# mittagessen/conformer_ocr

Measured on AMD Instinct MI355X. Metric: text lines/sec (whole node) + CER vs reference, 96×1200 bf16 batch, higher is better.
Workload: dtype bf16; 1 GPU; cfg2: conformer D=256 L=12 heads=4 sub_ch=256, batch 32 x 96x1200 per GPU, forward + CTC greedy; batches_in_queue=1, parallelism=1 independent rank(s), weights by one RCCL broadcast, streams_per_gpu=4, hipgraph_replay=True, launched_by=in-process, gpu_max_hw_queues=4, gpu_max_hw_queues_preset_by_caller=True

## Files before the change

conformer_ocr_amd/csrc/attention.hip.h:

```cpp
#pragma once
#include "common.hip.h"

__device__ __forceinline__ int xcd_remap_i(int bid, int nwg) {
    const int q = nwg >> 3, r = nwg & 7, xcd = bid & 7;
    return (xcd < r ? xcd * (q + 1) : r * (q + 1) + (xcd - r) * q) + (bid >> 3);
}

__device__ __forceinline__ float max3_f(float a, float b, float c) {
    float r;
    asm("v_max3_f32 %0, %1, %2, %3" : "=v"(r) : "v"(a), "v"(b), "v"(c));
    return r;
}

#define COCR_MFMA_WAIT "s_nop 7\n\ts_nop 7\n\ts_nop 3"
__device__ __forceinline__ void mfma_results_fence(f32x4 (&a)[4]) { asm volatile(COCR_MFMA_WAIT : "+v"(a[0]), "+v"(a[1]), "+v"(a[2]), "+v"(a[3])); }
__device__ __forceinline__ void mfma_results_fence(f32x4 (&a)[4], f32x4 (&b)[4]) {
    asm volatile(COCR_MFMA_WAIT : "+v"(a[0]), "+v"(a[1]), "+v"(a[2]), "+v"(a[3]), "+v"(b[0]), "+v"(b[1]), "+v"(b[2]), "+v"(b[3]));
}
__device__ __forceinline__ void mfma_results_fence(f32x4 (&a)[4], f32x4 (&b)[4], f32x4 (&c)[4]) {
    asm volatile(COCR_MFMA_WAIT : "+v"(a[0]), "+v"(a[1]), "+v"(a[2]), "+v"(a[3]), "+v"(b[0]), "+v"(b[1]), "+v"(b[2]), "+v"(b[3]), "+v"(c[0]), "+v"(c[1]), "+v"(c[2]),
                 "+v"(c[3]));
}

#ifndef COCR_ATT_EXP
// ... 385 lines not shown
                if (i0 + row < Tn) *reinterpret_cast<bf16x8 *>(ctx + ((size_t)b * Tn + i0 + row) * (heads * DHP) + hh * DHP + 8 * ch) = v8;
            }
            return;
        }
    }
    if (dh == DHP) {
        if (i0 + il < Tn) {
            T *dst = ctx + ((size_t)b * Tn + i0 + il) * (heads * DHP) + hh * DHP + 4 * g;
#pragma unroll
            for (int d = 0; d < DT; ++d) {
                const f32x4 r4 = o[d] * inv;
                if constexpr (sizeof(T) == 2) { bf16x4 w = {(T)r4[0], (T)r4[1], (T)r4[2], (T)r4[3]}; *reinterpret_cast<bf16x4 *>(dst + 16 * d) = w; }
                else { *reinterpret_cast<f32x4 *>(dst + 16 * d) = r4; }
            }
        }
    } else if (i0 + il < Tn) {
        T *dst = ctx + ((size_t)b * Tn + i0 + il) * (heads * dh) + hh * dh;
#pragma unroll
        for (int d = 0; d < DT; ++d) {
            const int dd = 16 * d + 4 * g;
            if (dd + 3 < dh && (dh & 3) == 0) {
                float r4[4] = {o[d][0] * inv, o[d][1] * inv, o[d][2] * inv, o[d][3] * inv};
                if constexpr (sizeof(T) == 2) { bf16x4 w = {(T)r4[0], (T)r4[1], (T)r4[2], (T)r4[3]}; *reinterpret_cast<bf16x4 *>(dst + dd) = w; }
                else { *reinterpret_cast<f32x4 *>(dst + dd) = (f32x4){r4[0], r4[1], r4[2], r4[3]}; }
            } else {
#pragma unroll
                for (int r = 0; r < 4; ++r)
                    if (dd + r < dh) dst[dd + r] = from_f32<T>(o[d][r] * inv);
            }
        }
    }
}


constexpr int AF_QT = 10;
constexpr int AF_TK = 320;
constexpr int AF_SK = 20;
#ifndef COCR_AF_TWOPART
#define COCR_AF_TWOPART 1
#endif
constexpr int AF_WAVES = 8;
constexpr int AF_SROWS = 32;
constexpr size_t AF_LDS = (size_t)(2 * AF_TK + 16 * AF_QT + AF_TK) * 128 + AF_WAVES * AF_SROWS * AF_SK * sizeof(float);
static_assert(AF_LDS <= 160 * 1024, "LDS of the resident attention kernel");

struct AttnFullState {
    bf16x8 qu[2][2], qv[2][2];
    f32x4 o[2][4], osum[2];
    float m_run[2];
};

template <int NT>
__device__ __forceinline__ void attn_full_tiles(const unsigned char *ks, const unsigned char *vs, const unsigned char *ps, float *sk,
                                                AttnFullState &st, int lb_first, int Tn, int Tk, int kg0, int lane, bool sync_after_first = false) {
    typedef bf16_t T;
    constexpr int KC = 2, DT = 4, RS = 128;
    const int il = lane & 15, g = lane >> 4;
    const int fo0 = ((g ^ (il & 7)) << 4), fo1 = (((4 + g) ^ (il & 7)) << 4);
    auto &qu = st.qu;
    auto &qv = st.qv;
    auto &o = st.o;
    auto &osum = st.osum;
    auto &m_run = st.m_run;
    bf16x8 ones;
#pragma unroll
    for (int j = 0; j < 8; ++j) ones[j] = il == 0 ? (T)1.0f : (T)0.0f;

    for (int j0 = 0; j0 < Tk; j0 += 64) {
        const bool first_tile = kg0 + j0 == 0;
        f32x4 sc[NT][4], keep[NT];
#pragma unroll
        for (int half = 0; half < 2; ++half) {
            const int js = j0 + 32 * half;
            bf16x8 bfr[NT + 2][KC];
            {
                const unsigned char *pb0 = ps + (size_t)(lb_first - 16 * (NT - 1) + js + il) * RS;
#pragma unroll
                for (int u = 0; u < NT + 2; ++u) {
                    if (half == 1 && u == 0) continue;
                    bfr[u][0] = *reinterpret_cast<const bf16x8 *>(pb0 + u * 16 * RS + fo0);
                    bfr[u][1] = *reinterpret_cast<const bf16x8 *>(pb0 + u * 16 * RS + fo1);
                }
            }
#pragma unroll
            for (int t = 0; t < NT; ++t) {
                const f32x4 negm = {-m_run[t], -m_run[t], -m_run[t], -m_run[t]};
#pragma unroll
                for (int ml = 0; ml < 3; ++ml) {
                    f32x4 rr;
                    if (half == 1 && ml == 0) rr = keep[t];
                    else {
                        rr = negm;
#pragma unroll
                        for (int c = 0; c < KC; ++c) rr = mma16(bfr[ml + (NT - 1 - t)][c], qv[t][c], rr);
                    }
                    if (half == 0 && ml == 2) keep[t] = rr;
#pragma unroll
                    for (int r = 0; r < 4; ++r) sk[((16 * ml + 4 * g + r) & (AF_SROWS - 1)) * AF_SK + il] = rr[r];
                    if (ml >= 1) {
#pragma unroll
                        for (int r = 0; r < 4; ++r) sc[t][2 * half + ml - 1][r] = sk[((15 - il + 16 * (ml - 1) + 4 * g + r) & (AF_SROWS - 1)) * AF_SK + il];
                    }
                }
            }
            bf16x8 kf[2][KC];
#pragma unroll
            for (int tl = 0; tl < 2; ++tl) {
                const unsigned char *kr = ks + (size_t)(js + 16 * tl + il) * RS;
                kf[tl][0] = *reinterpret_cast<const bf16x8 *>(kr + fo0);
                kf[tl][1] = *reinterpret_cast<const bf16x8 *>(kr + fo1);
            }
#pragma unroll
            for (int t = 0; t < NT; ++t)
#pragma unroll
                for (int tl = 0; tl < 2; ++tl)
#pragma unroll
                    for (int c = 0; c < KC; ++c) sc[t][2 * half + tl] = mma16(kf[tl][c], qu[t][c], sc[t][2 * half + tl]);
        }
        bf16x8 pb[NT][2];
        if constexpr (NT == 1) mfma_results_fence(sc[0]);
        else if constexpr (NT == 2) mfma_results_fence(sc[0], sc[1]);
// ... 51 lines not shown
                    for (int r = 0; r < 4; ++r) sc[t][tt][r] -= delta;
            }
        }
#pragma unroll
        for (int t = 0; t < NT; ++t) {
#pragma unroll
            for (int tt = 0; tt < 4; ++tt)
#pragma unroll
                for (int r = 0; r < 4; ++r) pb[t][tt >> 1][4 * (tt & 1) + r] = (T)__builtin_amdgcn_exp2f(sc[t][tt][r]);
            osum[t] = mma16(ones, pb[t][0], osum[t]);
            osum[t] = mma16(ones, pb[t][1], osum[t]);
        }
#pragma unroll
        for (int d = 0; d < DT; ++d) {
            const bf16x8 v0 = load_vt_frag<true>(vs, RS, j0, d, il, g, T()), v1 = load_vt_frag<true>(vs, RS, j0 + 32, d, il, g, T());
#pragma unroll
            for (int t = 0; t < NT; ++t) {
                o[t][d] = mma16(v0, pb[t][0], o[t][d]);
                o[t][d] = mma16(v1, pb[t][1], o[t][d]);
            }
        }
        if (j0 == 0 && sync_after_first) {
            asm volatile("s_waitcnt vmcnt(0)" ::: "memory");
            __builtin_amdgcn_s_barrier();
        }
    }
}

template <int NT>
__device__ __forceinline__ void attn_full_store(float *sk, const AttnFullState &st, bf16_t *ctxh, int ctx_stride, int i_first, int Tn, int lane) {
    typedef bf16_t T;
    constexpr int DT = 4;
    const int il = lane & 15, g = lane >> 4;
    auto &o = st.o;
    auto &osum = st.osum;
    unsigned char *stg = reinterpret_cast<unsigned char *>(sk);
#pragma unroll
    for (int t = 0; t < NT; ++t) {
        const float inv = 1.0f / __shfl(osum[t][0], il, 64);
#pragma unroll
        for (int d = 0; d < DT; ++d) {
            const f32x4 r4 = o[t][d] * inv;
            const bf16x4 w = {(T)r4[0], (T)r4[1], (T)r4[2], (T)r4[3]};
            *reinterpret_cast<bf16x4 *>(stg + il * 128 + (((2 * d + (g >> 1)) ^ (il & 7)) << 4) + 8 * (g & 1)) = w;
        }
#pragma unroll
        for (int j = 0; j < 2; ++j) {
            const int row = 8 * j + (lane >> 3), ch = lane & 7;
            const bf16x8 v8 = *reinterpret_cast<const bf16x8 *>(stg + row * 128 + ((ch ^ (row & 7)) << 4));
            const int i = i_first + 16 * t + row;
            if (i < Tn) *reinterpret_cast<bf16x8 *>(ctxh + (size_t)i * ctx_stride + 8 * ch) = v8;
        }
    }
}

template <bool LONG>
__global__ __launch_bounds__(64 * AF_WAVES) void relpos_attention_full_kernel(const bf16_t *__restrict__ q, const bf16_t *__restrict__ k, const bf16_t *__restrict__ v,
                                                                    const bf16_t *__restrict__ ptab, const float *__restrict__ ub,
                                                                    const float *__restrict__ vb, bf16_t *__restrict__ ctx,
                                                                    int Tn, int Tp, int heads, float scale, int pos_center, int ntw, int kpass) {
    typedef bf16_t T;
    extern __shared__ __attribute__((aligned(16))) unsigned char att_smem[];
    const int Tk = (Tn + 63) & ~63;
    const int Kp = min(kpass, Tk);
    const int nbr = 16 * ntw + Kp;
    unsigned char *ks = att_smem, *vs = ks + (size_t)Kp * 128, *ps = vs + (size_t)Kp * 128;
    float *skew = reinterpret_cast<float *>(ps + (size_t)nbr * 128);
    const int tid = threadIdx.x, lane = tid & 63;
    const int wave = __builtin_amdgcn_readfirstlane(tid >> 6);
    const int nqb = gridDim.x, logical = xcd_remap_i(blockIdx.x + nqb * blockIdx.y, nqb * gridDim.y);
    const int qb = logical % nqb, bh = logical / nqb, b = bh / heads, hh = bh - b * heads;
    const int i0 = qb * 16 * ntw;
    const int nt_here = min(ntw, (Tn - i0 + 15) >> 4);
    static_assert(AF_QT <= 2 * AF_WAVES, "at most two query tiles per wave");
    const int base = nt_here / AF_WAVES, extra = nt_here % AF_WAVES;
    const int mine = base + (wave < extra ? 1 : 0), first = wave * base + min(wave, extra);
    const int i_first = i0 + 16 * first;
    bf16x8 qq[2][2];
    f32x4 u4[2][2], v4[2][2];
    {
        const int il = lane & 15, g = lane >> 4;
        const T *qrows = q + (size_t)bh * Tp * 64;
#pragma unroll
        for (int t = 0; t < 2; ++t) {
            const int iq = min(i_first + 16 * min(t, max(mine - 1, 0)) + il, Tn - 1);
#pragma unroll
            for (int c = 0; c < 2; ++c) qq[t][c] = load_frag(qrows + (size_t)iq * 64 + c * 32 + 8 * g);
        }
#pragma unroll
        for (int c = 0; c < 2; ++c)
#pragma unroll
            for (int hlf = 0; hlf < 2; ++hlf) {
                u4[c][hlf] = *reinterpret_cast<const f32x4 *>(ub + hh * 64 + c * 32 + 8 * g + 4 * hlf);
                v4[c][hlf] = *reinterpret_cast<const f32x4 *>(vb + hh * 64 + c * 32 + 8 * g + 4 * hlf);
            }
    }
    auto stage = [&](int kg0, int a, int b2) {
        const int r8 = lane >> 3, cs = lane & 7, gch = (cs ^ r8) * 8;
        const T *kb = k + ((size_t)bh * Tp + kg0) * 64, *vbs = v + ((size_t)bh * Tp + kg0) * 64;
        for (int rg = a / 8 + wave; rg < b2 / 8; rg += AF_WAVES) {
            __builtin_amdgcn_global_load_lds((gbl_ptr_t)(kb + (size_t)(rg * 8 + r8) * 64 + gch), (lds_ptr_t)(ks + rg * 1024), 16, 0, 0);
            __builtin_amdgcn_global_load_lds((gbl_ptr_t)(vbs + (size_t)(rg * 8 + r8) * 64 + gch), (lds_ptr_t)(vs + rg * 1024), 16, 0, 0);
        }
        const int prow = heads * 64;
        const T *pb = ptab + (size_t)(pos_center - i0 - (16 * ntw - 1) + kg0) * prow + hh * 64;
        for (int rg = (a ? (16 * ntw + a) / 8 : 0) + wave; rg < (16 * ntw + b2) / 8; rg += AF_WAVES)
            __builtin_amdgcn_global_load_lds((gbl_ptr_t)(pb + (size_t)(rg * 8 + r8) * prow + gch), (lds_ptr_t)(ps + rg * 1024), 16, 0, 0);
    };
    stage(0, 0, (!LONG && COCR_AF_TWOPART) ? min(64, Kp) : Kp);
    AttnFullState st;
#pragma unroll
    for (int t = 0; t < 2; ++t) {
#pragma unroll
        for (int c = 0; c < 2; ++c)
#pragma unroll
            for (int j = 0; j < 8; ++j) {
                const float x = (float)qq[t][c][j];
                st.qu[t][c][j] = (T)((x + u4[c][j >> 2][j & 3]) * scale);
                st.qv[t][c][j] = (T)((x + v4[c][j >> 2][j & 3]) * scale);
            }
        st.osum[t] = (f32x4){0.f, 0.f, 0.f, 0.f};
        st.m_run[t] = 0.f;
#pragma unroll
        for (int d = 0; d < 4; ++d) st.o[t][d] = (f32x4){0.f, 0.f, 0.f, 0.f};
    }
    const int lb_first = 16 * ntw - 16 - 16 * first;
    float *sk = skew + wave * AF_SROWS * AF_SK;
    if constexpr (!LONG) {
        const bool two = COCR_AF_TWOPART && Kp > 64;
        asm volatile("s_waitcnt vmcnt(0)" ::: "memory");
        __builtin_amdgcn_s_barrier();
        if (two) stage(0, 64, Kp);
        if (mine == 0) {
            if (two) { asm volatile("s_waitcnt vmcnt(0)" ::: "memory"); __builtin_amdgcn_s_barrier(); }
            return;
        }
        T *ctxh = ctx + (size_t)b * Tn * (heads * 64) + hh * 64;
        if (mine == 1) { attn_full_tiles<1>(ks, vs, ps, sk, st, lb_first, Tn, Kp, 0, lane, two); attn_full_store<1>(sk, st, ctxh, heads * 64, i_first, Tn, lane); }
        else { attn_full_tiles<2>(ks, vs, ps, sk, st, lb_first, Tn, Kp, 0, lane, two); attn_full_store<2>(sk, st, ctxh, heads * 64, i_first, Tn, lane); }
        return;
    }
    for (int kg0 = 0; kg0 < Tk; kg0 += Kp) {
        const int kn = min(Kp, Tk - kg0);
        if (kg0 > 0) {
            __builtin_amdgcn_s_barrier();
            stage(kg0, 0, kn);
        }
        asm volatile("s_waitcnt vmcnt(0)" ::: "memory");
        __builtin_amdgcn_s_barrier();
        if (mine == 1) attn_full_tiles<1>(ks, vs, ps, sk, st, lb_first, Tn, kn, kg0, lane);
        else if (mine == 2) attn_full_tiles<2>(ks, vs, ps, sk, st, lb_first, Tn, kn, kg0, lane);
    }
    T *ctxh = ctx + (size_t)b * Tn * (heads * 64) + hh * 64;
    if (mine == 1) attn_full_store<1>(sk, st, ctxh, heads * 64, i_first, Tn, lane);
    else if (mine == 2) attn_full_store<2>(sk, st, ctxh, heads * 64, i_first, Tn, lane);
}

template <typename T, int DHP> static inline size_t attention_lds_bytes() {
    const size_t rb = DHP * sizeof(T);
    return (size_t)(64 + 64 + 128) * ((rb == 128 && sizeof(T) == 2) ? rb : rb + 16) + 4 * 48 * 20 * sizeof(float);
}
```

conformer_ocr_amd/csrc/cocr_api.hip:

```cpp
#include <hip/hip_runtime.h>

#include <algorithm>
#include <cmath>
#include <cstdarg>
#include <cstdio>
#include <cstdlib>
#include <cstring>
#include <map>
#include <string>
#include <thread>
#include <vector>

#include "../../include/cocr.h"
#include "attention.hip.h"
#include "common.hip.h"
#include "conv.hip.h"
#include "ctc.hip.h"
#include "ctc_loss.hip.h"
#include "train.hip.h"
#include "train_enc.hip.h"
#include "gemm.hip.h"
#include "ffn.hip.h"
#include "rowchain_args.hip.h"
#include "pack.hip.h"
// ... 93 lines not shown
    int dtype = -1;
    unsigned char *blob = nullptr;
    BlobPlan plan;
    unsigned char *packed = nullptr;
    bf16_t *fpack = nullptr;
    bool packed_stale = true;
    unsigned char *ptab = nullptr;
    size_t ptab_stride = 0;
    bool ptab_stale = true;
    cocr_model *owner = nullptr;
    unsigned long long wgen = 1, seen_wgen = 0;
    int capN = 0, capW = 0;
    std::vector<void *> ws_allocs;
    void *z_a = nullptr, *z_b = nullptr;
    float *x = nullptr;
    void *g_lines = nullptr;
    float *g_logits = nullptr;
    void *xn = nullptr, *hid = nullptr, *q = nullptr, *k = nullptr, *vt = nullptr, *ctx = nullptr, *glu = nullptr, *dwo = nullptr;
    size_t qkv_bytes = 0;
    int vtN = -1, vtT = -1;
    int pos_maxlen = COCR_POS_MAXLEN;
    DevBuf<unsigned char> pre_buf;
    DevBuf<unsigned char> page_buf;
    DevBuf<int32_t> d_lens, h_lens{true};
    int32_t *d_lens_cur = nullptr;
    int lens_slot = 0;
    DevBuf<int32_t> ctc_lab;
    DevBuf<float> ctc_val;
    const float *amax_logits = nullptr;
    int amax_rows = 0;
    bool amax_ok = false;
    DevBuf<float> tr_pad;
    DevBuf<unsigned char> beam_bp;
    DevBuf<int32_t> loss_d, loss_h{true};
    int loss_slot = 0;
    DevBuf<float> loss_ws;
    DevBuf<unsigned char> score_d, score_h{true};
    hipEvent_t score_ev[4] = {nullptr, nullptr, nullptr, nullptr};
    int score_slot = 0;
    DevBuf<unsigned> score_ws;
    int score_lds_max = 64 * 1024;
    int lastN = 0, lastT = 0;
    DevBuf<float> tr_part;
    float *tr_state = nullptr;
    long tr_step = 0;
    bool use_graph = false;
    struct GraphEntry { const void *lines; float *logits; int N, W, dtype; hipStream_t s; hipGraphExec_t exec; };
    std::vector<GraphEntry> graphs, graph_seen;
    bool debug = false;
    unsigned long long *stamps = nullptr;
    bool no_pad = false;
    bool beam_ref = false;
    bool no_front96 = false;
    bool no_front32 = false;
    bool no_dw_fuse = false;
    int chain_rows = 0;
    bool no_front_chain = false;
    bool ffn_probe = false;
    int att_resident_min = 192;
    bool att_resident_long = false;
    bool att_tiled = false;
    bool no_kskip = false;
    bool chain_xcd = true;
    bool no_chain = false;
    std::map<std::string, std::pair<float *, int64_t>> taps;
    DevBuf<float> tapbuf;
    TrainState *train = nullptr;
    bool profile = false;
    std::vector<ProfRec> prof;
    std::vector<hipEvent_t> ev_pool;
};

static const char *FAMILIES[] = {"frontend_fused", "frontend_conv12", "frontend_dw", "gemm_front_pw", "gemm_front_out", "layernorm",
                                 "gemm_ffn_up", "gemm_ffn_down", "ffn_fused", "chain_ffn_qkv", "chain_front_ffn_qkv", "chain_attn_out_glu", "chain_pw2_ffn_ffn_qkv", "chain_pw2_ffn", "gemm_qkv", "attention", "gemm_attn_out", "gemm_glu",
                                 "dwconv", "gemm_pw2", "gemm_decoder", "ctc_greedy", "ctc_beam", "ctc_loss", "ffn_probe", "event_pair_overhead"};
enum { FAM_FRONT96, FAM_CONV12, FAM_FDW, FAM_FPW, FAM_FOUT, FAM_LN, FAM_FFN_UP, FAM_FFN_DOWN, FAM_FFN_FUSED, FAM_CH_FIRST, FAM_CH_FRONT, FAM_CH_A, FAM_CH_B, FAM_CH_LAST, FAM_QKV, FAM_ATTN, FAM_AOUT, FAM_GLU,
       FAM_DW, FAM_PW2, FAM_DEC, FAM_GREEDY, FAM_BEAM, FAM_LOSS, FAM_FFN_PROBE, FAM_EMPTY, FAM_COUNT };

static void drop_graphs(cocr_model *m) {
    for (auto &g : m->graphs) (void)hipGraphExecDestroy(g.exec);
    m->graphs.clear();
    m->graph_seen.clear();
}

static int out_len1(int l) { return l >= 1 ? (l - 1) / 2 + 1 : 0; }

extern "C" int32_t cocr_out_len(int32_t in_len, int32_t subsampling_factor) {
    int n = 0;
    for (int f = subsampling_factor; f > 1; f >>= 1) ++n;
    for (int i = 0; i < n; ++i) in_len = out_len1(in_len);
    return in_len;
}

static void add_name(cocr_model *m, const std::string &n) { m->names.push_back(n); m->host[n]; }

struct Switch { const char *name; bool cocr_model::*flag; int cocr_model::*count; };
static const Switch SWITCHES[] = {
    {"COCR_NO_PAD", &cocr_model::no_pad, nullptr},
    {"COCR_NO_CHAIN", &cocr_model::no_chain, nullptr},
    {"COCR_NO_FRONT_CHAIN", &cocr_model::no_front_chain, nullptr},
    {"COCR_FFN_PROBE", &cocr_model::ffn_probe, nullptr},
    {"COCR_ATT_TILED", &cocr_model::att_tiled, nullptr},
    {"COCR_ATT_RESIDENT_LONG", &cocr_model::att_resident_long, nullptr},
    {"COCR_CHAIN_XCD", &cocr_model::chain_xcd, nullptr},
    {"COCR_NO_KSKIP", &cocr_model::no_kskip, nullptr},
    {"COCR_NO_DW_FUSE", &cocr_model::no_dw_fuse, nullptr},
    {"COCR_NO_FRONT96", &cocr_model::no_front96, nullptr},
    {"COCR_NO_FRONT32", &cocr_model::no_front32, nullptr},
    {"COCR_BEAM_REF", &cocr_model::beam_ref, nullptr},
    {"COCR_ATT_RESIDENT_MIN", nullptr, &cocr_model::att_resident_min},
    {"COCR_CHAIN_ROWS", nullptr, &cocr_model::chain_rows},
    {"COCR_SCORE_LDS_MAX", nullptr, &cocr_model::score_lds_max},
};

extern "C" int cocr_create(const cocr_hparams *hp, int device, cocr_model **out) {
    if (!hp || !out) return fail(COCR_EINVAL, "null argument");
    if (hp->num_classes < 1 || hp->height < 1 || hp->encoder_dim < 1 || hp->num_encoder_layers < 1 || hp->num_attention_heads < 1)
        return fail(COCR_EINVAL, "non-positive hyper-parameter");
    if (hp->encoder_dim % hp->num_attention_heads) return fail(COCR_EINVAL, "d_model %% num_heads should be zero.");
    if ((hp->conv_kernel_size - 1) % 2 || hp->conv_kernel_size < 1) return fail(COCR_EINVAL, "kernel_size should be a odd number for 'SAME' padding");
    if (hp->conv_expansion_factor != 2) return fail(COCR_EINVAL, "Currently, Only Supports expansion_factor 2");
    int sf = hp->subsampling_factor, snum = 0;
    if (sf < 2 || (sf & (sf - 1))) return fail(COCR_EINVAL, "Sampling factor should be a power of 2.");
    for (int f = sf; f > 1; f >>= 1) ++snum;
    if (snum < 1) return fail(COCR_EINVAL, "subsampling_factor must be at least 2");
    if (hp->encoder_dim % 16) return fail(COCR_EUNSUPPORTED, "encoder_dim must be a multiple of 16 (GLU tile pairing, 16-byte rows)");
    if (hp->subsampling_conv_channels % 8) return fail(COCR_EUNSUPPORTED, "subsampling_conv_channels must be a multiple of 8");
    if (hp->encoder_dim > COCR_LN_MAX_D) return fail(COCR_EUNSUPPORTED, "encoder_dim > 1024");
    const int dh = hp->encoder_dim / hp->num_attention_heads;
    if (dh > 128) return fail(COCR_EUNSUPPORTED, "d_head > 128");
    cocr_model *m = new cocr_model();
    m->hp = *hp;
    m->device = device;
    m->D = hp->encoder_dim; m->C = hp->subsampling_conv_channels; m->L = hp->num_encoder_layers;
    m->heads = hp->num_attention_heads; m->dh = dh; m->dhp = round_up(dh, 32);
    m->ff = hp->feed_forward_expansion_factor * hp->encoder_dim; m->ksz = hp->conv_kernel_size;
    m->rD = m->D; m->rff = m->ff; m->rdh = m->dh;
    m->ncls = hp->num_classes; m->H = hp->height; m->snum = snum;
    for (const Switch &w : SWITCHES) {
        const char *e = getenv(w.name);
        if (!e) continue;
        if (w.count) m->*w.count = atoi(e);
        else m->*w.flag = m->*w.flag ? e[0] != '0' : e[0] == '1';
    }
    { const char *e = getenv("COCR_CHAIN_STAMPS"); if (e && e[0] == '1') { (void)hipHostMalloc((void **)&m->stamps, 4096 * 8); memset(m->stamps, 0, 4096 * 8); } }
    int f = hp->height;
    for (int i = 0; i < snum; ++i) { f = out_len1(f); m->feats.push_back(f); }
    char buf[256];
    add_name(m, "encoder.conv_subsample.conv.0.weight");
    add_name(m, "encoder.conv_subsample.conv.0.bias");
    for (int s = 0, idx = 2; s < snum - 1; ++s, idx += 3) {
        for (int j = 0; j < 2; ++j) {
            snprintf(buf, sizeof buf, "encoder.conv_subsample.conv.%d.weight", idx + j); add_name(m, buf);
            snprintf(buf, sizeof buf, "encoder.conv_subsample.conv.%d.bias", idx + j); add_name(m, buf);
        }
    }
    add_name(m, "encoder.conv_subsample.out.0.weight");
    add_name(m, "encoder.conv_subsample.out.0.bias");
    for (int l = 0; l < m->L; ++l) {
        auto nm = [&](const char *suffix) { snprintf(buf, sizeof buf, "encoder.layers.%d.sequential.%s", l, suffix); add_name(m, buf); };
// ... 660 lines not shown
template <typename T> struct Fwd {
    cocr_model *m;
    const Form &f;
    hipStream_t s;
    const BlobPlan &P;
    const int N, W, D, T1, T2, F1, F2, Tn, M, Tp;
    const float ffr, scale;
    T *const za, *const zb;
    float *const x;
    T *const xn, *const hid, *const q, *const k, *const v, *const ctx, *const glu, *const dwo;
    Fwd(cocr_model *m_, const Form &f_, int N_, int W_, hipStream_t s_)
        : m(m_), f(f_), s(s_), P(m_->plan), N(N_), W(W_), D(m_->D), T1(out_len1(W_)), T2(m_->snum == 1 ? T1 : out_len1(T1)), F1(m_->feats[0]),
          F2(m_->feats[m_->snum == 1 ? 0 : 1]), Tn(cocr_out_len(W_, m_->hp.subsampling_factor)), M(N_ * Tn), Tp(round_up(Tn, 64)),
          ffr(m_->hp.half_step_residual ? 0.5f : 1.0f), scale(1.0f / sqrtf((float)m_->rdh)), za((T *)m_->z_a), zb((T *)m_->z_b), x(m_->x),
          xn((T *)m_->xn), hid((T *)m_->hid), q((T *)m_->q), k((T *)m_->k), v((T *)m_->vt), ctx((T *)m_->ctx), glu((T *)m_->glu), dwo((T *)m_->dwo) {}
    const float *F32(size_t off) const { return (const float *)(m->blob + off); }
    const T *WT(size_t off) const { return (const T *)(m->blob + off); }
    template <typename S> int tap(int l, const char *what, const S *src, size_t n) const {
        if (!f.taps) return COCR_OK;
        char nm[64];
        if (l < 0) snprintf(nm, sizeof nm, "%s", what);
        else snprintf(nm, sizeof nm, "l%d.%s", l, what);
        return ::tap<S>(m, s, nm, src, n);
    }
    int tap_x(int l, const char *what, const float *src) const { return tap<float>(l, what, src, (size_t)M * D); }
    int tap_qkv(int l) const {
        const size_t n = m->qkv_bytes / sizeof(T);
        int rc;
        if ((rc = tap<T>(l, "q", q, n)) || (rc = tap<T>(l, "k", k, n)) || (rc = tap<T>(l, "v", v, n))) return rc;
        return COCR_OK;
    }
};

template <typename T, typename TIn> static int frontend(const Fwd<T> &c, const TIn *lines) {
    cocr_model *m = c.m;
    const BlobPlan &P = c.P;
    const hipStream_t s = c.s;
    const int N = c.N, H = m->H, W = c.W, C = m->C, T1 = c.T1, F1 = c.F1, T2 = c.T2, F2 = c.F2;
    const FrontForm form = c.f.front;
    T *za = c.za, *zb = c.zb;
    int rc;
    if (form == FRONT_CONV0) {
        ProfScope ps(m, s, FAM_CONV12);
        const size_t npos = (size_t)N * T1 * F1;
        hipLaunchKernelGGL((frontend_conv0_kernel<T, TIn>), dim3((unsigned)((npos * (size_t)(C / 2) + 255) / 256)), dim3(256), 0, s, lines, H, W, T1, F1, C, npos,
                           c.F32(P.w0), c.F32(P.b0), zb);
        LAUNCH_CHECK();
        return COCR_OK;
    }
    if (form == FRONT_96) {
        ProfScope ps(m, s, FAM_FRONT96);
        const size_t n0 = (size_t)(C / 16) * 64 * 4;
        GEMM_TRY(launch_frontend96<TIn>(s, lines, N, H, W, T1, F1, T2, m->fpack, c.F32(P.b0), m->fpack + n0, c.F32(P.stages[0].dw_b),
                                        (const bf16_t *)(m->packed + P.stages[0].pw_w), c.F32(P.stages[0].pw_b), (bf16_t *)zb, m->stamps ? m->stamps + 128 : nullptr));
    } else if (form == FRONT_PW32) {
        ProfScope ps(m, s, FAM_CONV12);
        const size_t lds = (size_t)(4 * 16 + 3) * ((H + 11) & ~3) * 4 + (size_t)16 * F2 * 80;
        auto kern = frontend_conv12pw32_kernel<TIn>;
        GEMM_TRY(raise_lds_limit((const void *)kern, lds));
        hipLaunchKernelGGL(kern, dim3(ceil_div(T2, 16), N), dim3(256), lds, s, lines, H, W, T1, F1, T2, F2, c.F32(P.w0), c.F32(P.b0),
                           c.F32(P.stages[0].dw_w), c.F32(P.stages[0].dw_b), (const bf16_t *)c.WT(P.stages[0].pw_w), c.F32(P.stages[0].pw_b), (bf16_t *)zb);
        LAUNCH_CHECK();
    } else {
        {
            ProfScope ps(m, s, FAM_CONV12);
            if (form == FRONT_MFMA) {
                GEMM_TRY(launch_conv12_mfma<TIn>(s, lines, N, H, W, T1, F1, T2, F2, C, c.F32(P.w0), c.F32(P.b0), c.F32(P.stages[0].dw_w), c.F32(P.stages[0].dw_b),
                                                 (bf16_t *)za));
            } else {
                const int TB = std::max(1, 512 / C);
                const size_t lds = (size_t)(4 * TB + 3) * ((H + 11) & ~3) * 4;
                hipLaunchKernelGGL((frontend_conv12_kernel<T, TIn>), dim3(ceil_div(T2, TB), N), dim3(256), lds, s, lines, H, W, T1, F1, T2, F2, C,
                                   c.F32(P.w0), c.F32(P.b0), c.F32(P.stages[0].dw_w), c.F32(P.stages[0].dw_b), za, TB);
                LAUNCH_CHECK();
            }
        }
        if ((rc = c.tap(-1, "front.z2", za, (size_t)N * T2 * F2 * C))) return rc;
        ProfScope ps(m, s, FAM_FPW);
        EpiBiasAct<T, ACT_RELU> epi{zb, C, c.F32(P.stages[0].pw_b), C};
        GEMM_TRY(launch_gemm<T>(s, za, C, c.WT(P.stages[0].pw_w), C, N * T2 * F2, C, C, epi));
    }
    if ((rc = c.tap(-1, "front.z3", zb, (size_t)N * T2 * F2 * C))) return rc;
    int Tc = T2, Fc = F2;
    for (int st = 1; st < m->snum - 1; ++st) {
        const int To = out_len1(Tc), Fo = m->feats[st + 1];
        {
            ProfScope ps(m, s, FAM_FDW);
            hipLaunchKernelGGL((dw3x3s2_kernel<T>), dim3(1024), dim3(256), 0, s, zb, N, Tc, Fc, To, Fo, C, c.F32(P.stages[st].dw_w),
                               c.F32(P.stages[st].dw_b), za);
            LAUNCH_CHECK();
        }
        {
            ProfScope ps(m, s, FAM_FPW);
            EpiBiasAct<T, ACT_RELU> epi{zb, C, c.F32(P.stages[st].pw_b), C};
            GEMM_TRY(launch_gemm<T>(s, za, C, c.WT(P.stages[st].pw_w), C, N * To * Fo, C, C, epi));
        }
        Tc = To; Fc = Fo;
    }
    return COCR_OK;
}

template <typename T> static int layernorm(const Fwd<T> &c, size_t g1, size_t b1, bool write_f32, long g2, long b2) {
    ProfScope ps(c.m, c.s, FAM_LN);
    launch_layernorm<T>(c.s, c.x, c.M, c.D, c.F32(g1), c.F32(b1), write_f32 ? c.x : nullptr, g2 >= 0 ? c.F32((size_t)g2) : nullptr,
                        b2 >= 0 ? c.F32((size_t)b2) : nullptr, c.xn, c.m->rD);
    LAUNCH_CHECK();
    return COCR_OK;
// ... 993 lines not shown
```

conformer_ocr_amd/csrc/frontend.hip.h:

```cpp
#pragma once
#include "gemm.hip.h"
#include "conv.hip.h"

__global__ __launch_bounds__(256) void frontend_pack_kernel(const float *__restrict__ w0, const float *__restrict__ w2, bf16_t *__restrict__ w0f,
                                                            bf16_t *__restrict__ dwf, int C) {
    const int i = blockIdx.x * 256 + threadIdx.x;
    if (i < (C / 16) * 64 * 4) {
        const int e = i & 3, lane = (i >> 2) & 63, nt = i >> 8, r = lane & 15, g = lane >> 4;
        w0f[i] = (bf16_t)((g < 3 && e < 3) ? w0[(16 * nt + r) * 9 + 3 * g + e] : 0.0f);
    }
    if (i < (C / 16) * 5 * 64 * 8) {
        const int e = i & 7, lane = (i >> 3) & 63, chunk = (i >> 9) % 5, blk = i / (5 * 512), r = lane & 15, g = lane >> 4;
        const int tap = 2 * chunk + (g >> 1), cc = 8 * (g & 1) + e;
        dwf[i] = (bf16_t)((cc == r && tap < 9) ? w2[(16 * blk + r) * 9 + tap] : 0.0f);
    }
}

typedef unsigned u32x2_t __attribute__((ext_vector_type(2)));
__device__ __forceinline__ unsigned relu_pack2(float a, float b) {
    typedef short s16x2_t __attribute__((ext_vector_type(2)));
    typedef float f32x2_t __attribute__((ext_vector_type(2)));
    const bf16x2 h = __builtin_convertvector((f32x2_t){a, b}, bf16x2);
    const s16x2_t zero = {0, 0};
    return __builtin_bit_cast(unsigned, __builtin_elementwise_max(__builtin_bit_cast(s16x2_t, h), zero));
}
__device__ __forceinline__ u32x2_t relu_bf16x4(const f32x4 &v) { return (u32x2_t){relu_pack2(v[0], v[1]), relu_pack2(v[2], v[3])}; }

template <typename TIn>
__global__ __launch_bounds__(512) void frontend96_kernel(const TIn *__restrict__ X, int H, int W, int T1, int F1, int Tn,
                                                         const bf16_t *__restrict__ w0f, const float *__restrict__ b0,
                                                         const bf16_t *__restrict__ dwf, const float *__restrict__ b2,
                                                         const bf16_t *__restrict__ wpw,
                                                         const float *__restrict__ bpw, bf16_t *__restrict__ Z3, int HS, int N, unsigned long long *stamps) {
    typedef bf16_t T;
    constexpr int C = 256, F = 24, TB = 4, BMC = TB * F, MT = 6, KC1 = C / 32;
    constexpr int NA = 2 * TB + 1, NCOL = 4 * TB + 4, ZR = 2 * F + 2, ZC = 72;
    constexpr int PANEL = BMC * 128, IMG = 4 * PANEL, OS = C * 2 + 16, SLICE = 16 * 512;
    constexpr int XAB = BMC * OS > IMG ? BMC * OS : IMG;
    static_assert(BMC == 96, "operand image of the chain kernels");
    extern __shared__ __attribute__((aligned(16))) unsigned char smem[];
    unsigned char *xa = smem;
    T *z1 = reinterpret_cast<T *>(smem + XAB);
    T *xs = z1 + (NA * ZR + 1) * ZC;
    unsigned char *prm = reinterpret_cast<unsigned char *>(xs + NCOL * HS);
    const T *w0s = reinterpret_cast<const T *>(prm);
    const float *b0s = reinterpret_cast<const float *>(prm + 8192), *b2s = b0s + 256;

    const int tid = threadIdx.x, lane = tid & 63;
    const int wave = __builtin_amdgcn_readfirstlane(tid >> 6);
    const int r16 = lane & 15, g = lane >> 4, swz = r16 & 7;
    const int nblk = (Tn + TB - 1) / TB, nitems = nblk * N, stride = gridDim.x;
    int item = blockIdx.x;
#ifdef COCR_CHAIN_STAMPS_BUILD
    int nstamp = 0;
    auto stamp = [&]() {
        if (stamps && blockIdx.x == 1 && tid == 0 && nstamp < 40) stamps[nstamp] = __builtin_readcyclecounter();
        ++nstamp;
    };
#else
    auto stamp = [&]() {};
#endif
    stamp();

    constexpr int FILL = 4;
    TIn fv[FILL];
    auto load_pixels = [&](int it) {
        const int bb = it / nblk, c0 = 4 * (it - bb * nblk) * TB - 3;
        const TIn *Xb = X + (size_t)bb * H * W;
        int tv = tid;
        asm volatile("" : "+v"(tv));
#pragma unroll
        for (int u = 0; u < FILL; ++u) {
            const int i = tv + 512 * u, rr = i / NCOL, ci = i - rr * NCOL;
            const int w = min(max(c0 + ci, 0), W - 1), r = min(max(rr - 1, 0), H - 1);
            fv[u] = Xb[(size_t)r * W + w];
        }
    };
    if (item < nitems) load_pixels(item);
    __builtin_amdgcn_global_load_lds((gbl_ptr_t)(w0f + wave * 512 + lane * 8), (lds_ptr_t)(prm + wave * 1024), 16, 0, 0);
    if (wave < 2) __builtin_amdgcn_global_load_lds((gbl_ptr_t)((wave ? b2 : b0) + lane * 4), (lds_ptr_t)(prm + 8192 + wave * 1024), 16, 0, 0);
    asm volatile("s_waitcnt vmcnt(0)" ::: "memory");
    const int FT = (F1 + 15) >> 4, ntile = NA * FT;
    const int blk = wave & 3, mq = wave >> 2;

    for (; item < nitems; item += stride) {
    const int b = item / nblk, t0 = (item - b * nblk) * TB;
    int tv = tid;
    asm volatile("" : "+v"(tv));
    bf16x8 ring[16];
    for (int i = tv; i < NA * ZC; i += 512) {
        const int a = i / ZC, c = i - a * ZC;
        z1[(a * ZR) * ZC + c] = (T)0.0f;
        for (int zr = F1 + 1; zr < ZR; ++zr) z1[(a * ZR + zr) * ZC + c] = (T)0.0f;
    }
#pragma unroll
    for (int u = 0; u < FILL; ++u) {
        const int i = tv + 512 * u, rr = i / NCOL, ci = i - rr * NCOL, c = 4 * t0 - 3 + ci;
        const bool inside = c >= 0 && c < W && rr >= 1 && rr <= H;
        if (i < NCOL * HS) xs[ci * HS + rr] = (T)(inside ? pixel_to_f32<TIn>(fv[u]) : 0.0f);
    }
    stamp();
    asm volatile("s_waitcnt lgkmcnt(0)" ::: "memory");
    __builtin_amdgcn_s_barrier();
    stamp();

    s16x4 pf[4];
    bool valid[4];
    int zoff[4];
#pragma unroll
    for (int u = 0; u < 4; ++u) {
        const int mt = min(wave + 8 * u, ntile - 1);
        const int a = mt / FT, f1 = 16 * (mt - a * FT) + r16;
        const int t1 = 2 * t0 - 1 + a;
        const T *px = xs + (2 * a + g) * HS + 2 * f1;
        typedef unsigned u32x2 __attribute__((ext_vector_type(2)));
        pf[u] = __builtin_bit_cast(s16x4, (u32x2){*reinterpret_cast<const unsigned *>(px), *reinterpret_cast<const unsigned *>(px + 2)});
        valid[u] = t1 >= 0 && t1 < T1 && f1 < F1;
        zoff[u] = (wave + 8 * u < ntile && f1 + 1 < ZR) ? (a * ZR + f1 + 1) * ZC : NA * ZR * ZC;
    }
    const bool all_valid = __builtin_amdgcn_ballot_w64(valid[0] && valid[1] && valid[2] && valid[3]) == ~0ull;
    bf16x8 dwn[5];
    auto request_dw = [&](int pass) {
#pragma unroll
        for (int ch = 0; ch < 5; ++ch) dwn[ch] = *reinterpret_cast<const bf16x8 *>(dwf + ((size_t)(4 * pass + blk) * 5 + ch) * 512 + lane * 8);
    };
    request_dw(0);
    auto do_pass = [&](int pass, auto LAST) {
        const int cb = 64 * pass;
        bf16x8 dwb[5];
#pragma unroll
        for (int ch = 0; ch < 5; ++ch) dwb[ch] = dwn[ch];
        if (pass < 3) request_dw(pass + 1);
        const f32x4 bias2 = *reinterpret_cast<const f32x4 *>(b2s + cb + 16 * blk + 4 * g);
        s16x4 wf[4];
        f32x4 bias0[4];
#pragma unroll
        for (int nt = 0; nt < 4; ++nt) {
            wf[nt] = *reinterpret_cast<const s16x4 *>(w0s + ((size_t)((cb >> 4) + nt) * 64 + lane) * 4);
            bias0[nt] = *reinterpret_cast<const f32x4 *>(b0s + cb + 16 * nt + 4 * g);
        }
        f32x4 c0[4][4];
#pragma unroll
        for (int u = 0; u < 4; ++u)
#pragma unroll
            for (int nt = 0; nt < 4; ++nt) c0[u][nt] = __builtin_amdgcn_mfma_f32_16x16x16bf16_1k(wf[nt], pf[u], bias0[nt], 0, 0, 0);
        auto z1_epilogue = [&](auto MASKED) {
#pragma unroll
            for (int u = 0; u < 4; ++u)
#pragma unroll
                for (int nt = 0; nt < 4; ++nt) {
                    typedef unsigned u32x2 __attribute__((ext_vector_type(2)));
                    u32x2 ob = relu_bf16x4(c0[u][nt]);
                    if (decltype(MASKED)::value && !valid[u]) ob = (u32x2){0u, 0u};
                    *reinterpret_cast<u32x2 *>(z1 + zoff[u] + 16 * nt + 4 * g) = ob;
                }
        };
        if (all_valid) z1_epilogue(std::false_type{}); else z1_epilogue(std::true_type{});
        if constexpr (decltype(LAST)::value) {
            const T *first = wpw + (size_t)wave * SLICE;
#pragma unroll
            for (int f = 0; f < 16; ++f) ring[f] = *reinterpret_cast<const bf16x8 *>(first + f * 512 + lane * 8);
            if (item + stride < nitems) load_pixels(item + stride);
        }
        stamp();
        asm volatile("s_waitcnt lgkmcnt(0)" ::: "memory");
        __builtin_amdgcn_s_barrier();
        stamp();
#pragma unroll
        for (int u = 0; u < 3; ++u) {
            const int p = 16 * (mq + 2 * u) + r16, tl = p / F, f = p - tl * F;
            f32x4 acc = bias2;
#pragma unroll
            for (int ch = 0; ch < 5; ++ch) {
                const int tap = min(2 * ch + (g >> 1), 8), dt = tap / 3, df = tap - 3 * dt;
                const bf16x8 za = *reinterpret_cast<const bf16x8 *>(z1 + ((2 * tl + dt) * ZR + 2 * f + df) * ZC + 16 * blk + 8 * (g & 1));
                acc = mma16(dwb[ch], za, acc);
            }
            const bf16x4 o = {(T)acc[0], (T)acc[1], (T)acc[2], (T)acc[3]};
            const int col = cb + 16 * blk + 4 * g;
            *reinterpret_cast<bf16x4 *>(xa + (col >> 6) * PANEL + p * 128 + ((((col & 63) >> 3) ^ (p & 7)) << 4) + ((col & 7) >> 2) * 8) = o;
        }
        stamp();
        asm volatile("s_waitcnt lgkmcnt(0)" ::: "memory");
        __builtin_amdgcn_s_barrier();
    };
#pragma unroll 1
    for (int pass = 0; pass < 3; ++pass) do_pass(pass, std::false_type{});
    do_pass(3, std::true_type{});

    const f32x4 bp0 = *reinterpret_cast<const f32x4 *>(bpw + 32 * wave + 4 * g), bp1 = *reinterpret_cast<const f32x4 *>(bpw + 32 * wave + 16 + 4 * g);
    f32x4 acc[MT][2];
#pragma unroll
    for (int i = 0; i < MT; ++i) { acc[i][0] = bp0; acc[i][1] = bp1; }
#pragma unroll
    for (int kk = 0; kk < KC1; ++kk) {
        bf16x8 a[MT];
#pragma unroll
        for (int i = 0; i < MT; ++i) a[i] = lds_frag_swz(xa + (kk >> 1) * PANEL + (16 * i + r16) * 128, kk & 1, g, swz, T());
#pragma unroll
        for (int j = 0; j < 2; ++j)
#pragma unroll
            for (int i = 0; i < MT; ++i) acc[i][j] = mma16(ring[2 * kk + j], a[i], acc[i][j]);
    }
    stamp();
    __builtin_amdgcn_s_barrier();
    unsigned char *tile = xa;
#pragma unroll
    for (int j = 0; j < 2; ++j)
#pragma unroll
        for (int i = 0; i < MT; ++i) {
            const int row = 16 * i + r16;
            typedef unsigned u32x2 __attribute__((ext_vector_type(2)));
            *reinterpret_cast<u32x2 *>(tile + row * OS + (32 * wave + 16 * j + 4 * g) * 2) = relu_bf16x4(acc[i][j]);
        }
    asm volatile("s_waitcnt lgkmcnt(0)" ::: "memory");
    __builtin_amdgcn_s_barrier();
    stamp();
    T *out = Z3 + ((size_t)b * Tn + t0) * F * C;
    for (int id = tv; id < BMC * 32; id += 512) {
        const int row = id >> 5, ch = id & 31;
        if (t0 + row / F < Tn) copy16(out + (size_t)row * C + ch * 8, reinterpret_cast<const T *>(tile + row * OS + ch * 16));
    }
    stamp();
    }
}

static inline bool frontend96_supported(int C, int F1, int F2, int H) { return C == 256 && F2 == 24 && F1 <= 2 * F2 && H <= 4 * F2; }

template <typename TIn>
static inline hipError_t launch_frontend96(hipStream_t s, const TIn *X, int N, int H, int W, int T1, int F1, int Tn, const bf16_t *w0f, const float *b0,
                                           const bf16_t *dwf, const float *b2, const bf16_t *wpw, const float *bpw, bf16_t *Z3, unsigned long long *stamps = nullptr) {
    const int FT = (F1 + 15) / 16, HS = 2 * 16 * FT + 4;
    const size_t z1b = (size_t)(9 * 50 + 1) * 72 * 2, tileb = (size_t)96 * (256 * 2 + 16);
    const size_t lds = std::max((size_t)4 * 96 * 128, tileb) + z1b + (size_t)20 * HS * 2 + 10240;
    auto kern = frontend96_kernel<TIn>;
    hipError_t e = raise_lds_limit((const void *)kern, lds + 4096);
    if (e != hipSuccess) return e;
    static int ncu = 0;
    if (!ncu) {
        int dev = 0;
        hipDeviceProp_t prop;
        if (hipGetDevice(&dev) != hipSuccess || hipGetDeviceProperties(&prop, dev) != hipSuccess) return hipErrorUnknown;
        ncu = prop.multiProcessorCount > 0 ? prop.multiProcessorCount : 256;
    }
    const int nitems = ((Tn + 3) / 4) * N;
    hipLaunchKernelGGL(kern, dim3(std::min(nitems, ncu)), dim3(512), lds, s, X, H, W, T1, F1, Tn, w0f, b0, dwf, b2, wpw, bpw, Z3, HS, N, stamps);
    return hipGetLastError();
}
```

Baseline: 34780 lines/s.

## Split unbalanced attention query tiles across waves and preload frontend pointwise weights

In the resident attention kernel, when a block has one or two extra query tiles beyond one per wave, idle waves process the first half of the key range for an extra tile. They hand their partial softmax state (o, osum, running max) through LDS with a workgroup-scope flag, and the owning wave finishes the remaining keys. This balances work across waves at the cost of spin-waiting and extra LDS traffic. Separately, the frontend kernel now loads the pointwise weight ring once before the item loop (optionally per item under a new env flag) and issues the next depthwise weight request after the z1 epilogue rather than before it.

```diff
diff --git a/conformer_ocr_amd/csrc/attention.hip.h b/conformer_ocr_amd/csrc/attention.hip.h
--- a/conformer_ocr_amd/csrc/attention.hip.h
+++ b/conformer_ocr_amd/csrc/attention.hip.h
@@ -461,7 +461,8 @@
 
 template <int NT>
 __device__ __forceinline__ void attn_full_tiles(const unsigned char *ks, const unsigned char *vs, const unsigned char *ps, float *sk,
-                                                AttnFullState &st, int lb_first, int Tn, int Tk, int kg0, int lane, bool sync_after_first = false) {
+                                                AttnFullState &st, int lb_first, int Tn, int Tk, int kg0, int lane, bool sync_after_first = false,
+                                                int jb = 0) {
     typedef bf16_t T;
     constexpr int KC = 2, DT = 4, RS = 128;
     const int il = lane & 15, g = lane >> 4;
@@ -475,7 +476,7 @@
 #pragma unroll
     for (int j = 0; j < 8; ++j) ones[j] = il == 0 ? (T)1.0f : (T)0.0f;
 
-    for (int j0 = 0; j0 < Tk; j0 += 64) {
+    for (int j0 = jb; j0 < Tk; j0 += 64) {
         const bool first_tile = kg0 + j0 == 0;
         f32x4 sc[NT][4], keep[NT];
 #pragma unroll
@@ -633,6 +634,26 @@
             if (i < Tn) *reinterpret_cast<bf16x8 *>(ctxh + (size_t)i * ctx_stride + 8 * ch) = v8;
         }
     }
+}
+
+constexpr int AF_HAND_FLAG = (AF_SROWS - 1) * AF_SK + 16;
+static_assert(AF_HAND_FLAG * sizeof(float) >= 2048 && AF_HAND_FLAG < AF_SROWS * AF_SK, "flag behind the store's staging rows, inside the tile");
+__host__ __device__ constexpr int af_give_tiles(int nkt) { return (nkt + 1) / 2; }
+__device__ __forceinline__ void attn_full_give(unsigned char *buf, float *flag, const AttnFullState &st, int lane) {
+#pragma unroll
+    for (int d = 0; d < 4; ++d) *reinterpret_cast<f32x4 *>(buf + d * 1024 + lane * 16) = st.o[0][d];
+    *reinterpret_cast<f32x4 *>(buf + 4096 + lane * 16) = st.osum[0];
+    *reinterpret_cast<float *>(buf + 5120 + lane * 4) = st.m_run[0];
+    __hip_atomic_store(reinterpret_cast<unsigned *>(flag), 1u, __ATOMIC_RELEASE, __HIP_MEMORY_SCOPE_WORKGROUP);
+}
+__device__ __forceinline__ void attn_full_take(const unsigned char *buf, float *flag, AttnFullState &st, int lane) {
+    while (__hip_atomic_load(reinterpret_cast<unsigned *>(flag), __ATOMIC_ACQUIRE, __HIP_MEMORY_SCOPE_WORKGROUP) != 1u) __builtin_amdgcn_s_sleep(4);
+#pragma unroll
+    for (int d = 0; d < 4; ++d) st.o[0][d] = *reinterpret_cast<const f32x4 *>(buf + d * 1024 + lane * 16);
+    st.osum[0] = *reinterpret_cast<const f32x4 *>(buf + 4096 + lane * 16);
+    st.m_run[0] = *reinterpret_cast<const float *>(buf + 5120 + lane * 4);
+#pragma unroll
+    for (int c = 0; c < 2; ++c) { st.qu[0][c] = st.qu[1][c]; st.qv[0][c] = st.qv[1][c]; }
 }
 
 template <bool LONG>
@@ -657,6 +678,9 @@
     const int base = nt_here / AF_WAVES, extra = nt_here % AF_WAVES;
     const int mine = base + (wave < extra ? 1 : 0), first = wave * base + min(wave, extra);
     const int i_first = i0 + 16 * first;
+    const bool hand = !LONG && COCR_AF_TWOPART && Kp > 64 && base == 1 && extra >= 1 && extra <= 2;
+    const bool giver = hand && wave >= 4 && wave < 4 + extra, taker = hand && wave >= 6 && wave < 6 + extra;
+    const int handed = taker ? (wave - 2) + extra : first;
     bf16x8 qq[2][2];
     f32x4 u4[2][2], v4[2][2];
     {
@@ -664,7 +688,7 @@
         const T *qrows = q + (size_t)bh * Tp * 64;
 #pragma unroll
         for (int t = 0; t < 2; ++t) {
-            const int iq = min(i_first + 16 * min(t, max(mine - 1, 0)) + il, Tn - 1);
+            const int iq = min((t == 1 && taker ? i0 + 16 * handed : i_first + 16 * min(t, max(mine - 1, 0))) + il, Tn - 1);
 #pragma unroll
             for (int c = 0; c < 2; ++c) qq[t][c] = load_frag(qrows + (size_t)iq * 64 + c * 32 + 8 * g);
         }
@@ -709,7 +733,9 @@
     float *sk = skew + wave * AF_SROWS * AF_SK;
     if constexpr (!LONG) {
         const bool two = COCR_AF_TWOPART && Kp > 64;
-        asm volatile("s_waitcnt vmcnt(0)" ::: "memory");
+        float *flag = skew + (taker ? wave - 2 : wave) * AF_SROWS * AF_SK + AF_HAND_FLAG;
+        if (giver && lane == 0) __hip_atomic_store(reinterpret_cast<unsigned *>(flag), 0u, __ATOMIC_RELAXED, __HIP_MEMORY_SCOPE_WORKGROUP);
+        asm volatile("s_waitcnt vmcnt(0) lgkmcnt(0)" ::: "memory");
         __builtin_amdgcn_s_barrier();
         if (two) stage(0, 64, Kp);
         if (mine == 0) {
@@ -717,9 +743,17 @@
             return;
         }
         T *ctxh = ctx + (size_t)b * Tn * (heads * 64) + hh * 64;
-        if (mine == 1) { attn_full_tiles<1>(ks, vs, ps, sk, st, lb_first, Tn, Kp, 0, lane, two); attn_full_store<1>(sk, st, ctxh, heads * 64, i_first, Tn, lane); }
-        else { attn_full_tiles<2>(ks, vs, ps, sk, st, lb_first, Tn, Kp, 0, lane, two); attn_full_store<2>(sk, st, ctxh, heads * 64, i_first, Tn, lane); }
-        return;
+        if (mine == 2) { attn_full_tiles<2>(ks, vs, ps, sk, st, lb_first, Tn, Kp, 0, lane, two); attn_full_store<2>(sk, st, ctxh, heads * 64, i_first, Tn, lane); return; }
+        const int jsplit = 64 * af_give_tiles(Kp >> 6);
+        unsigned char *hbuf = (giver ? wave - 4 : wave - 6) ? vs : ks;
+        for (int round = 0;; ++round) {
+            const int tile = round ? handed : first;
+            attn_full_tiles<1>(ks, vs, ps, sk, st, 16 * ntw - 16 - 16 * tile, Tn, giver ? jsplit : Kp, 0, lane, two && round == 0, round ? jsplit : 0);
+            if (giver) { attn_full_give(hbuf, flag, st, lane); return; }
+            attn_full_store<1>(sk, st, ctxh, heads * 64, i0 + 16 * tile, Tn, lane);
+            if (!taker || round) return;
+            attn_full_take(hbuf, flag, st, lane);
+        }
     }
     for (int kg0 = 0; kg0 < Tk; kg0 += Kp) {
         const int kn = min(Kp, Tk - kg0);
diff --git a/conformer_ocr_amd/csrc/cocr_api.hip b/conformer_ocr_amd/csrc/cocr_api.hip
--- a/conformer_ocr_amd/csrc/cocr_api.hip
+++ b/conformer_ocr_amd/csrc/cocr_api.hip
@@ -169,6 +169,7 @@
     bool no_pad = false;
     bool beam_ref = false;
     bool no_front96 = false;
+    bool front_ring = false;
     bool no_front32 = false;
     bool no_dw_fuse = false;
     int chain_rows = 0;
@@ -223,6 +224,7 @@
     {"COCR_NO_KSKIP", &cocr_model::no_kskip, nullptr},
     {"COCR_NO_DW_FUSE", &cocr_model::no_dw_fuse, nullptr},
     {"COCR_NO_FRONT96", &cocr_model::no_front96, nullptr},
+    {"COCR_FRONT_RING", &cocr_model::front_ring, nullptr},
     {"COCR_NO_FRONT32", &cocr_model::no_front32, nullptr},
     {"COCR_BEAM_REF", &cocr_model::beam_ref, nullptr},
     {"COCR_ATT_RESIDENT_MIN", nullptr, &cocr_model::att_resident_min},
@@ -989,7 +991,8 @@
         ProfScope ps(m, s, FAM_FRONT96);
         const size_t n0 = (size_t)(C / 16) * 64 * 4;
         GEMM_TRY(launch_frontend96<TIn>(s, lines, N, H, W, T1, F1, T2, m->fpack, c.F32(P.b0), m->fpack + n0, c.F32(P.stages[0].dw_b),
-                                        (const bf16_t *)(m->packed + P.stages[0].pw_w), c.F32(P.stages[0].pw_b), (bf16_t *)zb, m->stamps ? m->stamps + 128 : nullptr));
+                                        (const bf16_t *)(m->packed + P.stages[0].pw_w), c.F32(P.stages[0].pw_b), (bf16_t *)zb, m->stamps ? m->stamps + 128 : nullptr,
+                                        m->front_ring));
     } else if (form == FRONT_PW32) {
         ProfScope ps(m, s, FAM_CONV12);
         const size_t lds = (size_t)(4 * 16 + 3) * ((H + 11) & ~3) * 4 + (size_t)16 * F2 * 80;
diff --git a/conformer_ocr_amd/csrc/frontend.hip.h b/conformer_ocr_amd/csrc/frontend.hip.h
--- a/conformer_ocr_amd/csrc/frontend.hip.h
+++ b/conformer_ocr_amd/csrc/frontend.hip.h
@@ -26,7 +26,7 @@
 }
 __device__ __forceinline__ u32x2_t relu_bf16x4(const f32x4 &v) { return (u32x2_t){relu_pack2(v[0], v[1]), relu_pack2(v[2], v[3])}; }
 
-template <typename TIn>
+template <typename TIn, bool RESIDENT = true>
 __global__ __launch_bounds__(512) void frontend96_kernel(const TIn *__restrict__ X, int H, int W, int T1, int F1, int Tn,
                                                          const bf16_t *__restrict__ w0f, const float *__restrict__ b0,
                                                          const bf16_t *__restrict__ dwf, const float *__restrict__ b2,
@@ -79,6 +79,12 @@
     if (item < nitems) load_pixels(item);
     __builtin_amdgcn_global_load_lds((gbl_ptr_t)(w0f + wave * 512 + lane * 8), (lds_ptr_t)(prm + wave * 1024), 16, 0, 0);
     if (wave < 2) __builtin_amdgcn_global_load_lds((gbl_ptr_t)((wave ? b2 : b0) + lane * 4), (lds_ptr_t)(prm + 8192 + wave * 1024), 16, 0, 0);
+    bf16x8 ring[16];
+    if constexpr (RESIDENT) {
+        const T *first = wpw + (size_t)wave * SLICE;
+#pragma unroll
+        for (int f = 0; f < 16; ++f) ring[f] = *reinterpret_cast<const bf16x8 *>(first + f * 512 + lane * 8);
+    }
     asm volatile("s_waitcnt vmcnt(0)" ::: "memory");
     const int FT = (F1 + 15) >> 4, ntile = NA * FT;
     const int blk = wave & 3, mq = wave >> 2;
@@ -87,7 +93,6 @@
     const int b = item / nblk, t0 = (item - b * nblk) * TB;
     int tv = tid;
     asm volatile("" : "+v"(tv));
-    bf16x8 ring[16];
     for (int i = tv; i < NA * ZC; i += 512) {
         const int a = i / ZC, c = i - a * ZC;
         z1[(a * ZR) * ZC + c] = (T)0.0f;
@@ -130,7 +135,6 @@
         bf16x8 dwb[5];
 #pragma unroll
         for (int ch = 0; ch < 5; ++ch) dwb[ch] = dwn[ch];
-        if (pass < 3) request_dw(pass + 1);
         const f32x4 bias2 = *reinterpret_cast<const f32x4 *>(b2s + cb + 16 * blk + 4 * g);
         s16x4 wf[4];
         f32x4 bias0[4];
@@ -156,10 +160,13 @@
                 }
         };
         if (all_valid) z1_epilogue(std::false_type{}); else z1_epilogue(std::true_type{});
+        if (pass < 3) request_dw(pass + 1);
         if constexpr (decltype(LAST)::value) {
-            const T *first = wpw + (size_t)wave * SLICE;
-#pragma unroll
-            for (int f = 0; f < 16; ++f) ring[f] = *reinterpret_cast<const bf16x8 *>(first + f * 512 + lane * 8);
+            if constexpr (!RESIDENT) {
+                const T *first = wpw + (size_t)wave * SLICE;
+#pragma unroll
+                for (int f = 0; f < 16; ++f) ring[f] = *reinterpret_cast<const bf16x8 *>(first + f * 512 + lane * 8);
+            }
             if (item + stride < nitems) load_pixels(item + stride);
         }
         stamp();
@@ -229,11 +236,12 @@
 
 template <typename TIn>
 static inline hipError_t launch_frontend96(hipStream_t s, const TIn *X, int N, int H, int W, int T1, int F1, int Tn, const bf16_t *w0f, const float *b0,
-                                           const bf16_t *dwf, const float *b2, const bf16_t *wpw, const float *bpw, bf16_t *Z3, unsigned long long *stamps = nullptr) {
+                                           const bf16_t *dwf, const float *b2, const bf16_t *wpw, const float *bpw, bf16_t *Z3, unsigned long long *stamps = nullptr,
+                                           bool ring_per_item = false) {
     const int FT = (F1 + 15) / 16, HS = 2 * 16 * FT + 4;
     const size_t z1b = (size_t)(9 * 50 + 1) * 72 * 2, tileb = (size_t)96 * (256 * 2 + 16);
     const size_t lds = std::max((size_t)4 * 96 * 128, tileb) + z1b + (size_t)20 * HS * 2 + 10240;
-    auto kern = frontend96_kernel<TIn>;
+    auto kern = ring_per_item ? frontend96_kernel<TIn, false> : frontend96_kernel<TIn, true>;
     hipError_t e = raise_lds_limit((const void *)kern, lds + 4096);
     if (e != hipSuccess) return e;
     static int ncu = 0;
```

Result: no change. 34570 lines/s (-0.6%).
